# penincillin/IHMR

Hardware: AMD Instinct MI355X
Metric: images/sec, IHMR-OPT 200-iter refinement batch=64 (ms/refine-iter: latency.ms_per_refine_iter; amortised: ms_per_refine_iter_amortised) (higher is better)
Workload: dtype f32

## Files before the change

ihmr_amd/csrc/ihmr_hip.hip:

```cpp
#include <math.h>
#include <stdio.h>
#include <stdlib.h>
#include <string.h>

#include <algorithm>
#include <atomic>
#include <mutex>
#include <vector>

#include "ihmr_common.h"
#include "mano_lbs.h"
#include "sdf_collision.h"
#include "preprocess.h"
#include "augment.h"
#include "render.h"
#include "mlp_infer.h"
#include "refine.h"
#include "encoder.h"
#include "encoder_bf16.h"
#include "evaluate.h"
#include "train.h"
#include "train_conv.h"
#include "copy_pack.h"
#include "launch_plan.h"
// ... 105 lines not shown
        jseg[j] = (int32_t)seg_q.size();
        for (int q = start[j]; q < start[j + 1]; q += LBS_SEG) seg_q.push_back(q);
    }
    jseg[NJ] = (int32_t)seg_q.size();
    seg_q.push_back((int32_t)wv.size());
    std::vector<int32_t> fsoa((size_t)3 * NFP, 0);
    for (int f = 0; f < NFP; ++f)
        for (int k = 0; k < 3; ++k) {
            const int32_t id = h->faces[(f < NF ? f : 0) * 3 + k];
            if (id < 0 || id >= NV) { delete m; return -1; }
            fsoa[(size_t)k * NFP + f] = id;
        }
    std::vector<uint32_t> fpk(NFP, 0u);
    for (int f = 0; f < NFP; ++f)
        fpk[f] = (uint32_t)fsoa[f] | ((uint32_t)fsoa[(size_t)NFP + f] << 10) | ((uint32_t)fsoa[(size_t)2 * NFP + f] << 20);
    std::vector<float> pd4, sd4, vt4;
    pack4(pd.data(), NPF, pd4);
    pack4(sd_t.data(), 10, sd4);
    pack4(vt.data(), 1, vt4);
    int rc = 0;
    rc |= upload_as(&m->pd4, pd4); rc |= upload_as(&m->sd4, sd4); rc |= upload_as(&m->vt4, vt4);
    rc |= upload(&m->v_template, vt); rc |= upload(&m->shapedirs_t, sd_t); rc |= upload(&m->posedirs, pd);
    rc |= upload(&m->J_template, J_t); rc |= upload(&m->J_shapedirs, J_sd); rc |= upload(&m->weights, wts);
    rc |= upload_as(&m->w4_w, w4w); rc |= upload(&m->w4_j, w4j);
    m->sparse4 = sparse4;
    rc |= upload(&m->pose_mean, pm); rc |= upload(&m->parents, par); rc |= upload(&m->depth, depth);
    rc |= upload(&m->tip_ids, tips); rc |= upload(&m->wj_start, start); rc |= upload(&m->wj_vert, wv);
    rc |= upload(&m->wj_w, ww); rc |= upload(&m->seg_q, seg_q); rc |= upload(&m->jseg_start, jseg); rc |= upload(&m->faces, fsoa); rc |= upload(&m->faces_pk, fpk); rc |= upload(&m->J_regressor, jr);
    m->max_depth = maxd;
    m->nnz = (int)wv.size();
    m->nseg = (int)seg_q.size() - 1;
    if (m->nseg > LBS_SEG_CAP) { ihmr_mano_destroy(m); return -1; }
    {
        const int dyn = m->nseg * 12 * (int)sizeof(float);
        hipError_t e1 = hipFuncSetAttribute((const void*)lbs_bwd1_kernel<true>, hipFuncAttributeMaxDynamicSharedMemorySize, dyn);
        hipError_t e2 = hipFuncSetAttribute((const void*)lbs_bwd1_kernel<false>, hipFuncAttributeMaxDynamicSharedMemorySize, dyn);
        if (e1 != hipSuccess || e2 != hipSuccess) { ihmr_mano_destroy(m); return (int)(e1 != hipSuccess ? e1 : e2); }
        int dev = 0, lds_max = 0;
        (void)hipGetDevice(&dev);
        (void)hipDeviceGetAttribute(&lds_max, hipDeviceAttributeMaxSharedMemoryPerBlock, dev);
        const void* tails[4] = {(const void*)opt_tail_kernel<true, true>, (const void*)opt_tail_kernel<true>, (const void*)opt_tail_kernel<false>,
                                (const void*)opt_tail_kernel_trans};
        m->tail_fits = 1;
        const int tail_dyn = opt_tail_dynamic_lds(m->nseg);
        for (const void* k : tails) {
            hipFuncAttributes fa;
            const int dyn_k = k == (const void*)opt_tail_kernel_trans ? 0 : tail_dyn;
            if (hipFuncGetAttributes(&fa, k) != hipSuccess || (long)fa.sharedSizeBytes + dyn_k > (long)lds_max ||
                (dyn_k && hipFuncSetAttribute(k, hipFuncAttributeMaxDynamicSharedMemorySize, dyn_k) != hipSuccess))
                m->tail_fits = 0;
        }
        (void)hipGetLastError();
    }
    if (rc) return rc;
    *out = m;
    return 0;
}

extern "C" int ihmr_mano_destroy(ihmr_mano* m) {
    if (!m) return 0;
    void* ptrs[] = {m->v_template, m->shapedirs_t, m->posedirs, m->J_template, m->J_shapedirs, m->weights, m->pose_mean,
                    m->parents, m->depth, m->tip_ids, m->wj_start, m->wj_vert, m->wj_w, m->faces, m->J_regressor, m->pd4, m->sd4, m->vt4, m->seg_q, m->jseg_start,
                    m->w4_w, m->w4_j, m->faces_pk};
    for (void* p : ptrs)
        if (p) (void)hipFree(p);
    delete m;
    return 0;
}

extern "C" int ihmr_mano_update_shapedirs(ihmr_mano* m, const float* shapedirs_host) {
    if (!m || !shapedirs_host) return -1;
    std::vector<float> jr((size_t)NJ * NV), vt(NV3), sd_t, J_t, J_sd;
    HIP_TRY(hipMemcpy(jr.data(), m->J_regressor, jr.size() * 4, hipMemcpyDeviceToHost));
    HIP_TRY(hipMemcpy(vt.data(), m->v_template, vt.size() * 4, hipMemcpyDeviceToHost));
    derive_shape_constants(jr.data(), vt.data(), shapedirs_host, sd_t, J_t, J_sd);
    HIP_TRY(hipMemcpy(m->shapedirs_t, sd_t.data(), sd_t.size() * 4, hipMemcpyHostToDevice));
    HIP_TRY(hipMemcpy(m->J_shapedirs, J_sd.data(), J_sd.size() * 4, hipMemcpyHostToDevice));
    std::vector<float> sd4;
    pack4(sd_t.data(), 10, sd4);
    HIP_TRY(hipMemcpy(m->sd4, sd4.data(), sd4.size() * 4, hipMemcpyHostToDevice));
    return 0;
}

extern "C" size_t ihmr_mano_workspace_bytes(int N) { return lbs_ws_bytes(N); }

static_assert(plan::SKIN_SMALL_MAX_HANDS == LBS_SMALL_MAX_HANDS && plan::BWD2_LDS_MIN_HANDS == LBS_B2_MIN_HANDS &&
              plan::PREP_SMALL_MAX_HANDS == SDF_PREP_SMALL_MAX_HANDS, "stage_plan.h restates the launch-form thresholds of the kernel headers");
template <bool TWO_HAND, int MODE>
static void lbs_skin_launch_mode(const ihmr_mano* m, int N, int B, float* verts, float* joints, const LbsWork& wk, float* pose_off, hipStream_t st) {
    const bool small = plan::skin_small(N);
    const int hg8 = 8 * (small ? LBS_HG_SMALL : LBS_HG);
    const dim3 skin_grid(8, 4 * ((N + hg8 - 1) / hg8));
    if (small) hipLaunchKernelGGL((lbs_skin_kernel<TWO_HAND, MODE, LBS_HG_SMALL>), skin_grid, dim3(LBS_THREADS), 0, st, *m, (const float*)wk.skel, N, B,
                                  verts, joints, wk.v_posed, pose_off);
    else hipLaunchKernelGGL((lbs_skin_kernel<TWO_HAND, MODE, LBS_HG>), skin_grid, dim3(LBS_THREADS), 0, st, *m, (const float*)wk.skel, N, B, verts,
                            joints, wk.v_posed, pose_off);
}
#define LBS_SKIN_FULL 0
#define LBS_SKIN_REUSE 1
#define LBS_SKIN_KEEP_P 2
#define LBS_SKIN_FULL_STORE_P 3
static_assert(plan::SKIN_FULL == LBS_SKIN_FULL && plan::SKIN_REUSE == LBS_SKIN_REUSE && plan::SKIN_KEEP_P == LBS_SKIN_KEEP_P &&
              plan::SKIN_FULL_STORE_P == LBS_SKIN_FULL_STORE_P, "stage_plan.h restates the skin modes");
static int g_force_full_skin = 0;
template <bool TWO_HAND>
static void lbs_skin_launch(const ihmr_mano* m, int mode, int N, int B, float* verts, float* joints, const LbsWork& wk, hipStream_t st) {
    if (g_force_full_skin && (mode == LBS_SKIN_KEEP_P || mode == LBS_SKIN_FULL_STORE_P)) mode = LBS_SKIN_FULL;
    if (mode == LBS_SKIN_REUSE) lbs_skin_launch_mode<TWO_HAND, LBS_MODE_REUSE>(m, N, B, verts, joints, wk, nullptr, st);
    else if (mode == LBS_SKIN_KEEP_P) lbs_skin_launch_mode<TWO_HAND, LBS_MODE_KEEP_P>(m, N, B, verts, joints, wk, wk.pose_off, st);
    else lbs_skin_launch_mode<TWO_HAND, LBS_MODE_FULL>(m, N, B, verts, joints, wk, mode == LBS_SKIN_FULL_STORE_P ? wk.pose_off : nullptr, st);
}
extern "C" int ihmr_debug_force_full_skin(int force) {
    const int prev = g_force_full_skin;
    g_force_full_skin = force ? 1 : 0;
    return prev;
}
static int g_force_generic_tail = 0;
extern "C" int ihmr_debug_force_generic_tail(int force) {
    const int prev = g_force_generic_tail;
    g_force_generic_tail = force ? 1 : 0;
    return prev;
}

static void lbs_forward_launch(const ihmr_mano* m, bool two_hand, const float* orient, const float* pose, const float* betas,
                               const float* trans, int N, int B, float* verts, float* joints, const LbsWork& wk, hipStream_t st) {
    if (two_hand) {
        hipLaunchKernelGGL(lbs_skel_kernel<true>, dim3(N), dim3(192), 0, st, *m, orient, pose, betas, trans, B, wk.skel, joints);
        lbs_skin_launch<true>(m, LBS_SKIN_FULL, N, B, verts, joints, wk, st);
    } else {
        hipLaunchKernelGGL(lbs_skel_kernel<false>, dim3(N), dim3(192), 0, st, *m, orient, pose, betas, trans, B, wk.skel, joints);
        lbs_skin_launch<false>(m, LBS_SKIN_FULL, N, B, verts, joints, wk, st);
    }
}

static int g_bwd2_streaming = 0;
extern "C" int ihmr_debug_force_lbs_bwd2_streaming(int force) {
    const int prev = g_bwd2_streaming;
    g_bwd2_streaming = force ? 1 : 0;
    return prev;
}

static void lbs_backward_launch(const ihmr_mano* m, bool two_hand, int N, int B, const float* d_verts, const float* d_joints,
                                float* d_orient, float* d_pose, float* d_betas, float* d_trans, int need_mask, const LbsWork& wk,
                                hipStream_t st, bool bwd1_done = false) {
    const size_t part_lds = (size_t)m->nseg * 12 * sizeof(float);
    if (bwd1_done) {}
    else if (two_hand)
        hipLaunchKernelGGL(lbs_bwd1_kernel<true>, dim3(N), dim3(LBS_THREADS), part_lds, st, *m, wk, B, d_verts, d_joints, d_orient,
                           d_betas, d_trans, need_mask);
    else
        hipLaunchKernelGGL(lbs_bwd1_kernel<false>, dim3(N), dim3(LBS_THREADS), part_lds, st, *m, wk, B, d_verts, d_joints, d_orient,
                           d_betas, d_trans, need_mask);
    if (need_mask & 2) {
        if (plan::bwd2_lds(N, g_bwd2_streaming)) hipLaunchKernelGGL(lbs_bwd2_lds_kernel, dim3((N + 63) / 64, LBS_KG), dim3(320), 0, st, *m, wk, N);
        else hipLaunchKernelGGL(lbs_bwd2_kernel, dim3(5, (N + 31) / 32, LBS_KG), dim3(64), 0, st, *m, wk, N);
        if (two_hand) hipLaunchKernelGGL(lbs_bwd3_kernel<true>, dim3(N), dim3(64), 0, st, wk, N, B, d_pose);
        else hipLaunchKernelGGL(lbs_bwd3_kernel<false>, dim3(N), dim3(64), 0, st, wk, N, B, d_pose);
    }
}

extern "C" int ihmr_mano_lbs_fwd(const ihmr_mano* m, const float* orient, const float* pose, const float* betas, int N,
                                 float* verts, float* joints, void* workspace, void* stream) {
    if (!m || N <= 0 || !workspace) return -1;
    lbs_forward_launch(m, false, orient, pose, betas, nullptr, N, 0, verts, joints, lbs_carve(workspace, N), (hipStream_t)stream);
    return (int)hipGetLastError();
}

extern "C" int ihmr_mano_lbs_bwd(const ihmr_mano* m, int N, const void* workspace, const float* d_verts, const float* d_joints,
                                 float* d_orient, float* d_pose, float* d_betas, int need_mask, void* stream) {
    if (!m || N <= 0 || !workspace) return -1;
    lbs_backward_launch(m, false, N, 0, d_verts, d_joints, d_orient, d_pose, d_betas, nullptr, need_mask,
                        lbs_carve(const_cast<void*>(workspace), N), (hipStream_t)stream);
    return (int)hipGetLastError();
}

static int device_cu_count(int* cus_out) {
    static std::atomic<int> cache[64];
    int dev = 0;
    HIP_TRY(hipGetDevice(&dev));
    int cus = cache[dev & 63].load(std::memory_order_relaxed);
    if (cus == 0) {
        HIP_TRY(hipDeviceGetAttribute(&cus, hipDeviceAttributeMultiprocessorCount, dev));
        if (cus <= 0) cus = 256;
        cache[dev & 63].store(cus, std::memory_order_relaxed);
    }
    *cus_out = cus;
    return 0;
}

extern "C" size_t ihmr_sdf_workspace_bytes(int B) { return sdf_ws_bytes(2 * B) + (size_t)2 * NFP * 4 * 4 + 256; }

static int g_collect_stats = 0;

static int sdf_launch(const VertLayout& vl, const int32_t* faces_r_soa, const int32_t* faces_l_soa, const uint32_t* fpk_r,
                      const uint32_t* fpk_l, int B, SdfWorkspace ws, float robustifier, float* loss, float* per_vert, float* origin, float* dval, bool dense, hipStream_t st) {
    if (B <= 0 || 2 * B > SDF_MAX_HANDS) return -1;
    const int prep = plan::prep_form(2 * B, dense);
    ws.fpk[0] = fpk_r; ws.fpk[1] = fpk_l; ws.B = B;
    const bool timed = g_timer != nullptr;
    hipEvent_t tcur;
    if (timed) { if (int rc = timed_begin(&tcur, st)) return rc; }
    if (prep == plan::PREP_DENSE)
        hipLaunchKernelGGL((sdf_prep_kernel<true, SDF_PREP_THREADS_LARGE>), dim3(2 * B), dim3(SDF_PREP_THREADS_LARGE), 0, st, vl, B, faces_r_soa,
                           faces_l_soa, ws, g_collect_stats);
    else if (prep == plan::PREP_SMALL)
        hipLaunchKernelGGL((sdf_prep_kernel<false, SDF_PREP_THREADS_SMALL>), dim3(2 * B), dim3(SDF_PREP_THREADS_SMALL), 0, st, vl, B, faces_r_soa,
                           faces_l_soa, ws, g_collect_stats);
    else
        hipLaunchKernelGGL((sdf_prep_kernel<false, SDF_PREP_THREADS_LARGE>), dim3(2 * B), dim3(SDF_PREP_THREADS_LARGE), 0, st, vl, B, faces_r_soa,
                           faces_l_soa, ws, g_collect_stats);
    int cus = 0;
    if (int rc = device_cu_count(&cus)) return rc;
    const int dist_blocks = SDF_DIST_WG_PER_CU * cus;
    if (timed) { if (int rc = timed_next(&tcur, IHMR_TIMED_SDF_PREP, st)) return rc; }
    int nblk = dist_blocks;
#ifdef IHMR_TUNING_BUILD
    if (const char* e = getenv("IHMR_DIST_BLOCKS_PER_SAMPLE")) nblk = std::max(64, std::min(dist_blocks, atoi(e) * B));
#endif
    if (g_collect_stats) hipLaunchKernelGGL(sdf_dist_kernel<true>, dim3(nblk), dim3(SDF_THREADS), 0, st, ws);
    else hipLaunchKernelGGL(sdf_dist_kernel<false>, dim3(nblk), dim3(SDF_THREADS), 0, st, ws);
    if (timed) { if (int rc = timed_next(&tcur, IHMR_TIMED_SDF_DIST, st)) return rc; (void)hipEventDestroy(tcur); }
    if (loss)
        hipLaunchKernelGGL(sdf_sample_kernel, dim3(B), dim3(SDF_SAMPLE_THREADS), 0, st, vl, ws, robustifier, loss, per_vert, origin,
                           dval, B);
    return (int)hipGetLastError();
}

__global__ void faces_to_soa_kernel(const int32_t* __restrict__ aos, int32_t* __restrict__ soa, uint32_t* __restrict__ packed, int* zero8) {
    if (zero8 && blockIdx.x == 0 && threadIdx.x < SDF_NZERO) sdf_zero_counter(zero8, (int)threadIdx.x);
    const int f = blockIdx.x * blockDim.x + threadIdx.x;
    if (f >= NFP) return;
    const int s = f < NF ? f : 0;
    uint32_t pk = 0;
    for (int k = 0; k < 3; ++k) {
        const int32_t id = min(max(aos[s * 3 + k], 0), NV - 1);
        soa[k * NFP + f] = id;
        pk |= (uint32_t)id << (10 * k);
    }
    packed[f] = pk;
}
struct FaceCopies { const int32_t *soa_r, *soa_l; const uint32_t *pk_r, *pk_l; };
static FaceCopies faces_to_workspace(const int32_t* faces_right, const int32_t* faces_left, void* workspace, int B, const SdfWorkspace& ws, hipStream_t st) {
    int32_t* soa = (int32_t*)((char*)workspace + sdf_ws_bytes(2 * B));
    uint32_t* pk = (uint32_t*)(soa + 6 * NFP);
    hipLaunchKernelGGL(faces_to_soa_kernel, dim3((NFP + 255) / 256), dim3(256), 0, st, faces_right, soa, pk, ws.inside_count);
    hipLaunchKernelGGL(faces_to_soa_kernel, dim3((NFP + 255) / 256), dim3(256), 0, st, faces_left, soa + 3 * NFP, pk + NFP, (int*)nullptr);
    return FaceCopies{soa, soa + 3 * NFP, pk, pk + NFP};
}

extern "C" int ihmr_sdf_collision_ex(const int32_t* faces_right, const int32_t* faces_left, const float* hand_verts, int B,
                                     float robustifier, const ihmr_sdf_options* options, float* loss, float* per_vert,
                                     float* origin_scale, float* dval, void* workspace, void* stream) {
    if (!workspace || B <= 0 || 2 * B > SDF_MAX_HANDS) return -1;
    hipStream_t st = (hipStream_t)stream;
    SdfWorkspace ws = sdf_carve(workspace, 2 * B);
    if (options) {
        ws.align_corners = options->align_corners ? 1 : 0;
        if (options->loss_divisor > 0.f) ws.loss_div = options->loss_divisor;
        ws.swap_xz = options->swap_xz ? 1 : 0;
    }
    const FaceCopies f = faces_to_workspace(faces_right, faces_left, workspace, B, ws, st);
    VertLayout vl{hand_verts, (long)2 * NV3, (long)NV3};
    return sdf_launch(vl, f.soa_r, f.soa_l, f.pk_r, f.pk_l, B, ws, robustifier, loss, per_vert, origin_scale, dval, false, st);
}

extern "C" int ihmr_sdf_collision(const int32_t* faces_right, const int32_t* faces_left, const float* hand_verts, int B,
                                  float robustifier, float* loss, float* per_vert, float* origin_scale, float* dval,
                                  void* workspace, void* stream) {
    return ihmr_sdf_collision_ex(faces_right, faces_left, hand_verts, B, robustifier, nullptr, loss, per_vert, origin_scale, dval,
                                 workspace, stream);
}

extern "C" int ihmr_sdf_dense_grid(const int32_t* faces_right, const int32_t* faces_left, const float* hand_verts, int B,
                                   float* phi, void* workspace, void* stream) {
    if (!workspace || B <= 0 || 2 * B > SDF_MAX_HANDS) return -1;
    hipStream_t st = (hipStream_t)stream;
    SdfWorkspace ws = sdf_carve(workspace, 2 * B);
    const FaceCopies f = faces_to_workspace(faces_right, faces_left, workspace, B, ws, st);
    VertLayout vl{hand_verts, (long)2 * NV3, (long)NV3};
    int rc = sdf_launch(vl, f.soa_r, f.soa_l, f.pk_r, f.pk_l, B, ws, 0.f, nullptr, nullptr, nullptr, nullptr, true, st);
    if (rc) return rc;
    for (int b = 0; b < B; ++b)
        for (int hnd = 0; hnd < 2; ++hnd)
            HIP_TRY(hipMemcpyAsync(phi + ((size_t)b * 2 + hnd) * SDF_NVOX, ws.phi + ((size_t)hnd * B + b) * SDF_NVOX,
                                   (size_t)SDF_NVOX * 4, hipMemcpyDeviceToDevice, st));
    return (int)hipGetLastError();
}

extern "C" size_t ihmr_opt_workspace_bytes(int B) { return opt_ws_bytes(B); }

static const ParamStep kNoStep{0, 0.f, 0.f, 1.f, -1, 0, 0};
static SdfWorkspace opt_sdf_ws(const ihmr_opt_io* io, const OptWork& wk, int B, int lists, int static_mask) {
    SdfWorkspace ws = sdf_carve(wk.sdf_ws, 2 * B, true);
    const plan::SdfFlags f = plan::plan_sdf_flags(lists, static_mask, io->sdf_no_candidate_lists, io->sdf_no_static_reuse);
    ws.list_mode = f.list_mode;
    ws.force_rebuild = f.force_rebuild;
    ws.static_stage = f.static_stage;
    ws.static_mask = f.static_mask;
    ws.moving_box = f.moving_box;
    ws.align_corners = io->sdf_align_corners ? 1 : 0;
    if (io->sdf_loss_divisor > 0.f) ws.loss_div = io->sdf_loss_divisor;
    ws.swap_xz = io->sdf_swap_xz ? 1 : 0;
    return ws;
}

struct OptCtx {
    const ihmr_mano *m, *m_left;
// ... 656 lines not shown
}

extern "C" int ihmr_render_meshes(const float* verts, const int32_t* faces, const int32_t* csr_offsets, const int32_t* csr_ids, int n_verts,
                                  int n_faces, int face_split, const uint8_t* present, const float* albedo, const float* cam,
                                  const ihmr_render_lights* lights, const uint8_t* background, int S, uint8_t* out_img,
                                  int32_t* out_face_ids, void* workspace, int B, void* stream) {
    if (!verts || !faces || !csr_offsets || !csr_ids || !albedo || !cam || !lights || !out_img || !workspace) return -1;
    if (B <= 0 || B > 65535 || n_verts <= 0 || n_faces <= 0 || n_faces > (1 << 24) || n_verts > (1 << 24) || face_split < 0 ||
        face_split > n_faces || S < 16 || S > 2048)
        return -1;
    if ((uintptr_t)workspace & 3u) return -1;
    const hipStream_t st = (hipStream_t)stream;
    rnd_vertex* ws = static_cast<rnd_vertex*>(workspace);
    hipLaunchKernelGGL(render_vertex_kernel, dim3((n_verts + RND_THREADS - 1) / RND_THREADS, B), dim3(RND_THREADS), 0, st, verts, faces,
                       csr_offsets, csr_ids, n_verts, n_faces, face_split, albedo, cam, *lights, S, ws);
    const int tiles = (S + RND_TILE - 1) / RND_TILE;
    const int vec = S % RND_PPT == 0 && !((uintptr_t)out_img & 3u) && !((uintptr_t)background & 3u);
    hipLaunchKernelGGL(render_raster_kernel, dim3(tiles * tiles, B), dim3(RND_THREADS), 0, st, ws, faces, n_verts, n_faces, face_split,
                       present, background, S, vec, out_img, out_face_ids);
    return (int)hipGetLastError();
}

extern "C" int ihmr_draw_keypoints(uint8_t* img, const float* kps, const float* weight, const uint8_t* colour, int B, int S, int K,
                                   void* stream) {
    if (!img || !kps || !weight || !colour || B <= 0 || S <= 0 || S > 4096 || K <= 0) return -1;
    hipLaunchKernelGGL(draw_keypoints_kernel, dim3(B), dim3(RND_KP_THREADS), 0, (hipStream_t)stream, img, kps, weight, (int)colour[0],
                       (int)colour[1], (int)colour[2], S, K);
    return (int)hipGetLastError();
}

extern "C" int ihmr_copy_segments(const ihmr_copy_seg* segs, int n, void* stream) {
    if (!segs || n <= 0 || n > IHMR_COPY_MAX_SEGS) return -1;
    CopySegTable t;
    memset(&t, 0, sizeof(t));
    long biggest = 0;
    for (int i = 0; i < n; ++i) {
        const ihmr_copy_seg& g = segs[i];
        if (!g.src || !g.dst || g.rows <= 0 || g.width <= 0 || g.src_ld < g.width || g.dst_ld < g.width) return -1;
        if (((uintptr_t)g.src | (uintptr_t)g.dst) & 3u) return -1;
        t.s[i] = g;
        biggest = std::max(biggest, (long)g.rows * g.width);
    }
    const unsigned bx = (unsigned)std::max<long>(1, std::min<long>(64, (biggest + 1023) / 1024));
    hipLaunchKernelGGL(copy_segments_kernel, dim3(bx, (unsigned)n), dim3(256), 0, (hipStream_t)stream, t);
    return (int)hipGetLastError();
}

extern "C" int ihmr_root_align_joints(const float* joints4, float* out4, int B, void* stream) {
    if (!joints4 || !out4 || B <= 0) return -1;
    hipLaunchKernelGGL(root_align_joints_kernel, dim3(B), dim3(64), 0, (hipStream_t)stream, joints4, out4, B);
    return (int)hipGetLastError();
}

extern "C" int ihmr_set_kernel_timer(ihmr_kernel_timer* t) {
    std::lock_guard<std::mutex> lk(g_timer_mutex);
    g_timer = t;
    return 0;
}

extern "C" int ihmr_flush_kernel_timer(void) {
    std::lock_guard<std::mutex> lk(g_timer_mutex);
    for (auto& p : g_pending) {
        float ms = 0.f;
        HIP_TRY(hipEventSynchronize(p.b));
        HIP_TRY(hipEventElapsedTime(&ms, p.a, p.b));
        if (g_timer) {
            if (p.k < 0) { g_timer->ms_event_pair += ms; g_timer->n_event_pair += 1; }
            else if (p.k < IHMR_TIMED_KERNELS) { g_timer->ms[p.k] += ms; g_timer->n[p.k] += 1; }
        }
        (void)hipEventDestroy(p.a);
        (void)hipEventDestroy(p.b);
    }
    g_pending.clear();
    return 0;
}


#ifdef SDF_STAMPS
extern "C" int ihmr_debug_stamps(long long* host, int zero) {
    HIP_TRY(hipDeviceSynchronize());
    if (zero) {
        void* p; HIP_TRY(hipGetSymbolAddress(&p, HIP_SYMBOL(g_sdf_stamps))); HIP_TRY(hipMemset(p, 0, sizeof(long long) * 4096 * 4 * 8));
        HIP_TRY(hipGetSymbolAddress(&p, HIP_SYMBOL(g_sdf_prep))); HIP_TRY(hipMemset(p, 0, sizeof(long long) * 4096 * 8));
        return 0;
    }
    HIP_TRY(hipMemcpyFromSymbol(host, HIP_SYMBOL(g_sdf_stamps), sizeof(long long) * 4096 * 4 * 8));
    HIP_TRY(hipMemcpyFromSymbol(host + 4096 * 4 * 8, HIP_SYMBOL(g_sdf_span), sizeof(long long) * 4096 * 4 * 4));
    HIP_TRY(hipMemcpyFromSymbol(host + 4096 * 4 * 12, HIP_SYMBOL(g_sdf_prep), sizeof(long long) * 4096 * 8));
    return 0;
}
#endif

#ifdef SDF_QMASK_CHECK
extern "C" int ihmr_debug_sdf_ptrs(const ihmr_opt_io* io, int B, void** out4) {
    SdfWorkspace ws = sdf_carve(opt_carve(io->workspace, B).sdf_ws, 2 * B, true);
    out4[0] = ws.qcell; out4[1] = ws.inside_bits; out4[2] = ws.box; out4[3] = ws.phi;
    return 0;
}
extern "C" int ihmr_debug_qmask(unsigned* host8) {
    if (hipDeviceSynchronize() != hipSuccess) return -1;
    return (int)hipMemcpyFromSymbol(host8, HIP_SYMBOL(g_qmask_bad), 32);
}
#endif

#ifdef SDF_HANDLOG
extern "C" long ihmr_debug_handlog(unsigned* host, long cap) {
    static uint4* buf = nullptr;
    static unsigned cap_now = 0;
    if (hipDeviceSynchronize() != hipSuccess) return -1;
    if (cap > 0) {
        if (buf) (void)hipFree(buf);
        if (hipMalloc(&buf, (size_t)cap * 16) != hipSuccess) return -1;
        cap_now = (unsigned)cap;
        const unsigned zero = 0;
        if (hipMemcpyToSymbol(HIP_SYMBOL(g_handlog_n), &zero, 4) != hipSuccess) return -1;
        if (hipMemcpyToSymbol(HIP_SYMBOL(g_handlog_cap), &cap_now, 4) != hipSuccess) return -1;
        if (hipMemcpyToSymbol(HIP_SYMBOL(g_handlog), &buf, 8) != hipSuccess) return -1;
        return 0;
    }
    unsigned n = 0;
    if (hipMemcpyFromSymbol(&n, HIP_SYMBOL(g_handlog_n), 4) != hipSuccess) return -1;
    if (n > cap_now) n = cap_now;
    if (n && hipMemcpy(host, buf, (size_t)n * 16, hipMemcpyDeviceToHost) != hipSuccess) return -1;
    uint4* null = nullptr;
    (void)hipMemcpyToSymbol(HIP_SYMBOL(g_handlog), &null, 8);
    return (long)n;
}
#endif

#ifdef CONV_STAMPS
extern "C" int ihmr_debug_conv_stamps(long long* host, int zero) {
    HIP_TRY(hipDeviceSynchronize());
    void* p;
    HIP_TRY(hipGetSymbolAddress(&p, HIP_SYMBOL(g_conv_stamps)));
    if (zero) { HIP_TRY(hipMemset(p, 0, sizeof(long long) * 1024 * 10)); return 0; }
    HIP_TRY(hipMemcpy(host, p, sizeof(long long) * 1024 * 10, hipMemcpyDeviceToHost));
    return 0;
}
#endif

#ifdef TAIL_STAMPS
extern "C" int ihmr_debug_tail_stamps(long long* host, int zero) {
    HIP_TRY(hipDeviceSynchronize());
    void *p, *q;
    HIP_TRY(hipGetSymbolAddress(&p, HIP_SYMBOL(g_tail_stamps)));
    HIP_TRY(hipGetSymbolAddress(&q, HIP_SYMBOL(g_samp_stamps)));
    if (zero) { HIP_TRY(hipMemset(p, 0, sizeof(long long) * 3 * 4096 * 8)); HIP_TRY(hipMemset(q, 0, sizeof(long long) * 4096 * 8)); return 0; }
    HIP_TRY(hipMemcpy(host, p, sizeof(long long) * 3 * 4096 * 8, hipMemcpyDeviceToHost));
    HIP_TRY(hipMemcpy(host + 3 * 4096 * 8, q, sizeof(long long) * 4096 * 8, hipMemcpyDeviceToHost));
    return 0;
}
#endif

#ifdef IHMR_TIMELINE
extern "C" long ihmr_debug_timeline(unsigned long long* host, long cap) {
    static unsigned long long* ring = nullptr;
    static unsigned seg_cap = 0;
    if (hipDeviceSynchronize() != hipSuccess) return -1;
    void* cur = nullptr;
    if (hipGetSymbolAddress(&cur, HIP_SYMBOL(g_tl_cursor)) != hipSuccess) return -1;
    if (cap > 0) {
        if (ring) (void)hipFree(ring);
        seg_cap = (unsigned)(cap / 256);
        if (hipMalloc(&ring, (size_t)seg_cap * 256 * 24) != hipSuccess) return -1;
        if (hipMemset(cur, 0, 256 * 32 * 4) != hipSuccess) return -1;
        if (hipMemcpyToSymbol(HIP_SYMBOL(g_tl_cap), &seg_cap, 4) != hipSuccess) return -1;
        if (hipMemcpyToSymbol(HIP_SYMBOL(g_tl_ring), &ring, 8) != hipSuccess) return -1;
        return 0;
    }
    static unsigned counts[256 * 32];
    if (hipMemcpy(counts, cur, sizeof(counts), hipMemcpyDeviceToHost) != hipSuccess) return -1;
    long n = 0;
    for (int s = 0; s < 256; ++s) {
        const unsigned c = counts[s * 32] < seg_cap ? counts[s * 32] : seg_cap;
        if (c && hipMemcpy(host + 3 * n, ring + 3 * (size_t)s * seg_cap, (size_t)c * 24, hipMemcpyDeviceToHost) != hipSuccess) return -1;
        n += c;
    }
    unsigned long long* null = nullptr;
    (void)hipMemcpyToSymbol(HIP_SYMBOL(g_tl_ring), &null, 8);
    return n;
}
#endif

extern "C" const char* ihmr_version(void) { return "ihmr_hip 0.2 (gfx950)"; }
```

ihmr_amd/csrc/mano_lbs.h:

```cpp
#pragma once
#include "ihmr_common.h"

#define LBS_THREADS 256
#define LBS_HG 8
#define LBS_HG_SMALL 4
#define LBS_SMALL_MAX_HANDS 256
#define LBS_TILE_V 195
#define LBS_KG 25
#define LBS_KC 3
#define LBS_SEG 13
#define LBS_SEG_CAP 1024
#define LBS_CSR_CAP 4096

#define SK_R 0
#define SK_J 144
#define SK_G 192
#define SK_A 384
#define SK_PF 576
#define SK_POSE 712
#define SK_BETA 760
#define SK_SHIFT 770
#define SK_STRIDE 784

struct LbsWork {
// ... 724 lines not shown
            }
            if (nc > 0) {
                bw.dG[p][e] += acc;
                if (c == 3) bw.dJ[p][r] -= accJ;
            }
        }
        if (tid >= 192 && tid < 192 + NJ * 3) {
            const int j = (tid - 192) / 3, c = (tid - 192) % 3;
            if (bw.dep[j] == d) bw.dJ[j][c] += bw.drel[j][c];
        }
        __syncthreads();
    }
    if (tid < 9) bw.dR[0][tid] = bw.dG[0][4 * (tid / 3) + (tid % 3)];
    if (tid >= 64 && tid < 67) bw.dJ[0][tid - 64] += bw.dG[0][4 * (tid - 64) + 3];
    __syncthreads();

    if (need_orient && tid == 0) {
        float dr[3];
        rodrigues_bwd(bw.sk + SK_POSE, bw.dR[0], dr);
        if (left) { dr[1] = -dr[1]; dr[2] = -dr[2]; }
        d_orient[h * 3 + 0] = dr[0]; d_orient[h * 3 + 1] = dr[1]; d_orient[h * 3 + 2] = dr[2];
    }
    if (need_pose && tid < NJ * 9) wk.chain[(size_t)h * 192 + tid] = bw.dR[tid / 9][tid % 9];

    if (need_betas) {
        if (TWO_HAND) {
            __syncthreads();
            if (tid < 3) {
                if (!left) bw.dJ[0][tid] += bw.gsum[tid];
                else bw.dJ[0][tid] += tid == 0 ? bw.gsum[0] : -bw.gsum[tid];
            }
            __syncthreads();
        }
        const int wave = tid / WAVE, lane = tid % WAVE;
        if (IN_LDS) {
            for (int l = wave; l < 10; l += LBS_THREADS / WAVE) {
                float4 srow[NVP / WAVE];
#pragma unroll
                for (int t = 0; t < NVP / WAVE; ++t) srow[t] = m.sd4[l * NVP + lane + WAVE * t];
                __builtin_amdgcn_sched_barrier(0);
                float acc = 0.f;
#pragma unroll
                for (int t = 0; t < NVP / WAVE; ++t) {
                    const int v = lane + WAVE * t;
                    if (v < NV) {
                        acc = __builtin_fmaf(srow[t].x, bw.vp[3 * v], acc);
                        acc = __builtin_fmaf(srow[t].y, bw.vp[3 * v + 1], acc);
                        acc = __builtin_fmaf(srow[t].z, bw.vp[3 * v + 2], acc);
                    }
                }
                if (lane < 48) acc = __builtin_fmaf(m.J_shapedirs[lane * 10 + l], bw.dJ[lane / 3][lane % 3], acc);
                acc = wave_reduce_sum(acc);
                if (lane == 0) d_betas[h * 10 + l] = acc;
            }
            return;
        }
        const float* dvp_h = wk.dvp + (size_t)h * NV3;
        for (int l = wave; l < 10; l += LBS_THREADS / WAVE) {
            float acc = 0.f;
#pragma unroll
            for (int half = 0; half < 2; ++half) {
                constexpr int T0[2] = {0, 7}, T1[2] = {7, NVP / WAVE};
                float4 srow[7];
                float dv[7][3];
#pragma unroll
                for (int t = T0[half]; t < T1[half]; ++t) {
                    const int v = min(lane + WAVE * t, NV - 1);
                    srow[t - T0[half]] = m.sd4[l * NVP + lane + WAVE * t];
                    dv[t - T0[half]][0] = dvp_h[3 * v]; dv[t - T0[half]][1] = dvp_h[3 * v + 1]; dv[t - T0[half]][2] = dvp_h[3 * v + 2];
                }
                __builtin_amdgcn_sched_barrier(0);
#pragma unroll
                for (int t = T0[half]; t < T1[half]; ++t) {
                    if (lane + WAVE * t < NV) {
                        acc = __builtin_fmaf(srow[t - T0[half]].x, dv[t - T0[half]][0], acc);
                        acc = __builtin_fmaf(srow[t - T0[half]].y, dv[t - T0[half]][1], acc);
                        acc = __builtin_fmaf(srow[t - T0[half]].z, dv[t - T0[half]][2], acc);
                    }
                }
            }
            if (lane < 48) acc = __builtin_fmaf(m.J_shapedirs[lane * 10 + l], bw.dJ[lane / 3][lane % 3], acc);
            acc = wave_reduce_sum(acc);
            if (lane == 0) d_betas[h * 10 + l] = acc;
        }
    }
}

template <bool TWO_HAND>
__global__ __launch_bounds__(LBS_THREADS, 4) void lbs_bwd1_kernel(ihmr_mano m, LbsWork wk, int B,
                                                               const float* __restrict__ d_verts,
                                                               const float* __restrict__ d_joints,
                                                               float* __restrict__ d_orient, float* __restrict__ d_betas,
                                                               float* __restrict__ d_trans, int need_mask) {
    __shared__ LbsBwdShared bw;
    extern __shared__ __attribute__((aligned(16))) float bwd1_part[];
    lbs_bwd1_hand<TWO_HAND>(m, wk, B, (int)blockIdx.x, (int)threadIdx.x, bw, bwd1_part, d_verts, d_joints, d_orient, d_betas, d_trans, need_mask);
}

typedef float lbs_f32x16 __attribute__((ext_vector_type(16)));
__global__ __launch_bounds__(64) void lbs_bwd2_kernel(ihmr_mano m, LbsWork wk, int N) {
    TL_SCOPE(8);
    const int lane = threadIdx.x, l31 = lane & 31, kp = lane >> 5;
    const int e = blockIdx.x * 32 + l31, hand = blockIdx.y * 32 + l31, kg = blockIdx.z;
    const float* arow = m.posedirs + (size_t)min(e, NPF - 1) * NV3;
    const float* brow = wk.dvp + (size_t)min(hand, N - 1) * NV3;
    const bool a_ok = e < NPF, b_ok = hand < N;
    typedef float lbs_f4u __attribute__((ext_vector_type(4), aligned(8)));
    lbs_f4u av[LBS_KC][4], bv[LBS_KC][4];
#pragma unroll
    for (int c = 0; c < LBS_KC; ++c) {
        const int k0 = (kg * LBS_KC + c) * 32 + 16 * kp;
#pragma unroll
        for (int q = 0; q < 4; ++q) {
            const int k = min(k0 + 4 * q, NV3 - 4);
            av[c][q] = *reinterpret_cast<const lbs_f4u*>(arow + k);
            bv[c][q] = *reinterpret_cast<const lbs_f4u*>(brow + k);
        }
    }
    __builtin_amdgcn_sched_barrier(0);
    lbs_f32x16 acc;
#pragma unroll
    for (int r = 0; r < 16; ++r) acc[r] = 0.f;
#pragma unroll
    for (int c = 0; c < LBS_KC; ++c) {
        const int k0 = (kg * LBS_KC + c) * 32 + 16 * kp;
#pragma unroll
        for (int q = 0; q < 4; ++q) {
            const int kq = k0 + 4 * q;
            const bool sh = kq + 4 > NV3 && kq < NV3;
            const float ax[4] = {sh ? av[c][q].z : av[c][q].x, sh ? av[c][q].w : av[c][q].y, av[c][q].z, av[c][q].w};
            const float bx[4] = {sh ? bv[c][q].z : bv[c][q].x, sh ? bv[c][q].w : bv[c][q].y, bv[c][q].z, bv[c][q].w};
#pragma unroll
            for (int t = 0; t < 4; ++t) {
                const bool k_ok = kq + t < NV3;
                const float a0 = (a_ok && k_ok) ? ax[t] : 0.f, b0 = (b_ok && k_ok) ? bx[t] : 0.f;
                acc = __builtin_amdgcn_mfma_f32_32x32x2f32(a0, b0, acc, 0, 0, 0);
            }
        }
    }
    if (b_ok) {
        float* dst = wk.dpf_part + ((size_t)kg * N + hand) * 136 + blockIdx.x * 32 + 4 * kp;
#pragma unroll
        for (int r4 = 0; r4 < 4; ++r4) {
            const int e4 = blockIdx.x * 32 + 4 * kp + 8 * r4;
            if (e4 + 3 < 136) *reinterpret_cast<float4*>(dst + 8 * r4) = make_float4(acc[4 * r4], acc[4 * r4 + 1], acc[4 * r4 + 2], acc[4 * r4 + 3]);
        }
    }
}

#ifndef LBS_B2_MIN_HANDS
#define LBS_B2_MIN_HANDS 256
#endif
#define LBS_B2_LDK 33
#define LBS_B2_ROWS (160 + 64)
__global__ __launch_bounds__(320) void lbs_bwd2_lds_kernel(ihmr_mano m, LbsWork wk, int N) {
    TL_SCOPE(8);
    __shared__ float tile[2][LBS_B2_ROWS][LBS_B2_LDK];
    const int tid = threadIdx.x, lane = tid % WAVE, wave = tid / WAVE, l31 = lane & 31, kp = lane >> 5;
    const int h0 = blockIdx.x * 64, kg = blockIdx.y;
    float v4[6][4];
    auto load_chunk = [&](int c) {
        const int k0 = (kg * LBS_KC + c) * 32;
#pragma unroll
        for (int i = 0; i < 6; ++i) {
            const int u = tid + 320 * i, row = u >> 3, k = k0 + 4 * (u & 7);
            v4[i][0] = v4[i][1] = v4[i][2] = v4[i][3] = 0.f;
            if (row >= LBS_B2_ROWS) continue;
            const bool is_a = row < 160;
            const int r = is_a ? row : h0 + (row - 160);
            if (is_a ? r >= NPF : r >= N) continue;
            const float* src = (is_a ? m.posedirs + (size_t)r * NV3 : wk.dvp + (size_t)r * NV3) + k;
            if (k + 3 < NV3) {
                typedef float lbs_f4u __attribute__((ext_vector_type(4), aligned(4)));
                const lbs_f4u x = *reinterpret_cast<const lbs_f4u*>(src);
                v4[i][0] = x.x; v4[i][1] = x.y; v4[i][2] = x.z; v4[i][3] = x.w;
            } else {
#pragma unroll
                for (int t = 0; t < 4; ++t) v4[i][t] = k + t < NV3 ? src[t] : 0.f;
            }
        }
    };
    auto store_chunk = [&](int buf) {
#pragma unroll
        for (int i = 0; i < 6; ++i) {
            const int u = tid + 320 * i, row = u >> 3, kq = 4 * (u & 7);
            if (row >= LBS_B2_ROWS) continue;
#pragma unroll
            for (int t = 0; t < 4; ++t) tile[buf][row][kq + t] = v4[i][t];
        }
    };
    lbs_f32x16 acc0, acc1;
#pragma unroll
    for (int r = 0; r < 16; ++r) { acc0[r] = 0.f; acc1[r] = 0.f; }
    load_chunk(0);
    store_chunk(0);
    __syncthreads();
#pragma unroll 1
    for (int c = 0; c < LBS_KC; ++c) {
        const int cur = c & 1;
        if (c + 1 < LBS_KC) load_chunk(c + 1);
        const float* arow = &tile[cur][wave * 32 + l31][16 * kp];
        const float* b0row = &tile[cur][160 + l31][16 * kp];
        const float* b1row = &tile[cur][160 + 32 + l31][16 * kp];
#pragma unroll
        for (int st = 0; st < 16; ++st) {
            const float a = arow[st], b0 = b0row[st], b1 = b1row[st];
            acc0 = __builtin_amdgcn_mfma_f32_32x32x2f32(a, b0, acc0, 0, 0, 0);
            acc1 = __builtin_amdgcn_mfma_f32_32x32x2f32(a, b1, acc1, 0, 0, 0);
        }
        if (c + 1 < LBS_KC) store_chunk(cur ^ 1);
        __syncthreads();
    }
#pragma unroll
    for (int half = 0; half < 2; ++half) {
        const int hand = h0 + 32 * half + l31;
        if (hand >= N) continue;
        const lbs_f32x16& acc = half ? acc1 : acc0;
        float* dst = wk.dpf_part + ((size_t)kg * N + hand) * 136 + wave * 32 + 4 * kp;
#pragma unroll
        for (int r4 = 0; r4 < 4; ++r4) {
            const int e4 = wave * 32 + 4 * kp + 8 * r4;
            if (e4 + 3 < 136) *reinterpret_cast<float4*>(dst + 8 * r4) = make_float4(acc[4 * r4], acc[4 * r4 + 1], acc[4 * r4 + 2], acc[4 * r4 + 3]);
        }
    }
}

template <bool TWO_HAND>
__device__ __forceinline__ void lbs_bwd3_hand(const LbsWork& wk, int N, int B, float* __restrict__ d_pose, int h, int j, float* dpf, bool active = true) {
    float r[3] = {0.f, 0.f, 0.f}, chain[9];
    const int jj = min(max(j, 1), NJ - 1);
    if (active) {
#pragma unroll
        for (int t = 0; t < 3; ++t) {
            const int e = j + 64 * t;
            if (e >= 136) break;
            float part[LBS_KG];
#pragma unroll
            for (int c = 0; c < LBS_KG; ++c) part[c] = wk.dpf_part[((size_t)c * N + h) * 136 + e];
            __builtin_amdgcn_sched_barrier(0);
            float acc = 0.f;
#pragma unroll
            for (int c = 0; c < LBS_KG; ++c) acc += part[c];
            dpf[e] = acc;
        }
#pragma unroll
        for (int k = 0; k < 3; ++k) r[k] = wk.skel[(size_t)h * SK_STRIDE + SK_POSE + 3 * jj + k];
#pragma unroll
        for (int e = 0; e < 9; ++e) chain[e] = wk.chain[(size_t)h * 192 + 9 * jj + e];
    }
    __syncthreads();
    if (!active || j < 1 || j >= NJ) return;
    const bool left = TWO_HAND && h >= B;
    float dR[9], dr[3];
#pragma unroll
    for (int e = 0; e < 9; ++e) dR[e] = chain[e] + dpf[(j - 1) * 9 + e];
    rodrigues_bwd(r, dR, dr);
    if (left) { dr[1] = -dr[1]; dr[2] = -dr[2]; }
    float* dst = d_pose + (size_t)h * 45 + 3 * (j - 1);
    dst[0] = dr[0]; dst[1] = dr[1]; dst[2] = dr[2];
}
template <bool TWO_HAND>
__global__ __launch_bounds__(64) void lbs_bwd3_kernel(LbsWork wk, int N, int B, float* __restrict__ d_pose) {
    TL_SCOPE(9);
    __shared__ float dpf[192];
    lbs_bwd3_hand<TWO_HAND>(wk, N, B, d_pose, (int)blockIdx.x, (int)threadIdx.x, dpf);
}
```

Baseline: 29810.

## Retile LBS bwd2 LDS GEMM to 32 hands per block with staged output

Reworks the posedirs-by-dvp GEMM kernel to process 32 hands per workgroup with 4 waves instead of 64 hands with 5 waves. The 8 leftover pose-feature rows are computed by a 16x16x4 MFMA on two waves. Row pointers are precomputed and tail loads are clamped, and results are staged through LDS so the global writes are coalesced. This doubles the grid size for better CU occupancy at small batches, at the cost of re-reading posedirs per block and adding divergent work for the remainder rows.

```diff
diff --git a/ihmr_amd/csrc/ihmr_hip.hip b/ihmr_amd/csrc/ihmr_hip.hip
--- a/ihmr_amd/csrc/ihmr_hip.hip
+++ b/ihmr_amd/csrc/ihmr_hip.hip
@@ -281,7 +281,7 @@
         hipLaunchKernelGGL(lbs_bwd1_kernel<false>, dim3(N), dim3(LBS_THREADS), part_lds, st, *m, wk, B, d_verts, d_joints, d_orient,
                            d_betas, d_trans, need_mask);
     if (need_mask & 2) {
-        if (plan::bwd2_lds(N, g_bwd2_streaming)) hipLaunchKernelGGL(lbs_bwd2_lds_kernel, dim3((N + 63) / 64, LBS_KG), dim3(320), 0, st, *m, wk, N);
+        if (plan::bwd2_lds(N, g_bwd2_streaming)) hipLaunchKernelGGL(lbs_bwd2_lds_kernel, dim3((N + LBS_B2_HANDS - 1) / LBS_B2_HANDS, LBS_KG), dim3(256), 0, st, *m, wk, N);
         else hipLaunchKernelGGL(lbs_bwd2_kernel, dim3(5, (N + 31) / 32, LBS_KG), dim3(64), 0, st, *m, wk, N);
         if (two_hand) hipLaunchKernelGGL(lbs_bwd3_kernel<true>, dim3(N), dim3(64), 0, st, wk, N, B, d_pose);
         else hipLaunchKernelGGL(lbs_bwd3_kernel<false>, dim3(N), dim3(64), 0, st, wk, N, B, d_pose);
@@ -1244,6 +1244,17 @@
 }
 #endif
 
+#ifdef BWD2_STAMPS
+extern "C" int ihmr_debug_bwd2_stamps(long long* host, int zero) {
+    HIP_TRY(hipDeviceSynchronize());
+    void* p;
+    HIP_TRY(hipGetSymbolAddress(&p, HIP_SYMBOL(g_bwd2_stamps)));
+    if (zero) { HIP_TRY(hipMemset(p, 0, sizeof(long long) * 1024 * 8)); return 0; }
+    HIP_TRY(hipMemcpy(host, p, sizeof(long long) * 1024 * 8, hipMemcpyDeviceToHost));
+    return 0;
+}
+#endif
+
 #ifdef IHMR_TIMELINE
 extern "C" long ihmr_debug_timeline(unsigned long long* host, long cap) {
     static unsigned long long* ring = nullptr;
diff --git a/ihmr_amd/csrc/mano_lbs.h b/ihmr_amd/csrc/mano_lbs.h
--- a/ihmr_amd/csrc/mano_lbs.h
+++ b/ihmr_amd/csrc/mano_lbs.h
@@ -900,77 +900,111 @@
 #define LBS_B2_MIN_HANDS 256
 #endif
 #define LBS_B2_LDK 33
-#define LBS_B2_ROWS (160 + 64)
-__global__ __launch_bounds__(320) void lbs_bwd2_lds_kernel(ihmr_mano m, LbsWork wk, int N) {
+#define LBS_B2_HANDS 32
+#define LBS_B2_ROWS (128 + LBS_B2_HANDS + 8)
+#define LBS_B2_OLD 140
+typedef float lbs_f32x4 __attribute__((ext_vector_type(4)));
+#ifdef BWD2_STAMPS
+__device__ long long g_bwd2_stamps[1024][8];
+#define BWD2_TK(k) do { const long long now_ = (long long)__builtin_readcyclecounter(); tk_[k] += now_ - tk_prev_; tk_prev_ = now_; } while (0)
+#else
+#define BWD2_TK(k)
+#endif
+__global__ __launch_bounds__(256) void lbs_bwd2_lds_kernel(ihmr_mano m, LbsWork wk, int N) {
     TL_SCOPE(8);
-    __shared__ float tile[2][LBS_B2_ROWS][LBS_B2_LDK];
-    const int tid = threadIdx.x, lane = tid % WAVE, wave = tid / WAVE, l31 = lane & 31, kp = lane >> 5;
-    const int h0 = blockIdx.x * 64, kg = blockIdx.y;
-    float v4[6][4];
+    __shared__ __attribute__((aligned(16))) float tile[2][LBS_B2_ROWS][LBS_B2_LDK];
+    static_assert(LBS_B2_HANDS * LBS_B2_OLD <= 2 * LBS_B2_ROWS * LBS_B2_LDK, "the output tile reuses the chunk buffers");
+    const int tid = threadIdx.x, lane = tid % WAVE, l31 = lane & 31, kp = lane >> 5;
+    const int wave = __builtin_amdgcn_readfirstlane(tid / WAVE);
+    const int h0 = blockIdx.x * LBS_B2_HANDS, kg = blockIdx.y;
+#ifdef BWD2_STAMPS
+    long long tk_[8] = {0, 0, 0, 0, 0, 0, 0, 0}, tk_prev_ = (long long)__builtin_readcyclecounter();
+#endif
+    typedef float lbs_f4u __attribute__((ext_vector_type(4), aligned(4)));
+    const float* srow[6];
+    bool sok[6];
+#pragma unroll
+    for (int i = 0; i < 6; ++i) {
+        const int row = (tid + 256 * i) >> 3;
+        if (row < 128) { srow[i] = m.posedirs + (size_t)row * NV3; sok[i] = true; }
+        else if (row < 128 + LBS_B2_HANDS) { const int h = h0 + row - 128; srow[i] = wk.dvp + (size_t)min(h, N - 1) * NV3; sok[i] = h < N; }
+        else { const int e = row - LBS_B2_HANDS; srow[i] = m.posedirs + (size_t)min(e, NPF - 1) * NV3; sok[i] = e < NPF; }
+    }
+    lbs_f4u v4[6];
     auto load_chunk = [&](int c) {
-        const int k0 = (kg * LBS_KC + c) * 32;
+        const int k = (kg * LBS_KC + c) * 32 + 4 * (tid & 7), kc = min(k, NV3 - 4);
+#pragma unroll
+        for (int i = 0; i < 6; ++i)
+            if (i < 5 || wave == 0) v4[i] = *reinterpret_cast<const lbs_f4u*>(srow[i] + kc);
+    };
+    auto store_chunk = [&](int buf, int c) {
+        const int k = (kg * LBS_KC + c) * 32 + 4 * (tid & 7);
+        const bool sh = k + 4 > NV3 && k < NV3;
 #pragma unroll
         for (int i = 0; i < 6; ++i) {
-            const int u = tid + 320 * i, row = u >> 3, k = k0 + 4 * (u & 7);
-            v4[i][0] = v4[i][1] = v4[i][2] = v4[i][3] = 0.f;
-            if (row >= LBS_B2_ROWS) continue;
-            const bool is_a = row < 160;
-            const int r = is_a ? row : h0 + (row - 160);
-            if (is_a ? r >= NPF : r >= N) continue;
-            const float* src = (is_a ? m.posedirs + (size_t)r * NV3 : wk.dvp + (size_t)r * NV3) + k;
-            if (k + 3 < NV3) {
-                typedef float lbs_f4u __attribute__((ext_vector_type(4), aligned(4)));
-                const lbs_f4u x = *reinterpret_cast<const lbs_f4u*>(src);
-                v4[i][0] = x.x; v4[i][1] = x.y; v4[i][2] = x.z; v4[i][3] = x.w;
-            } else {
-#pragma unroll
-                for (int t = 0; t < 4; ++t) v4[i][t] = k + t < NV3 ? src[t] : 0.f;
-            }
+            if (i == 5 && wave != 0) continue;
+            const float x[4] = {sh ? v4[i].z : v4[i].x, sh ? v4[i].w : v4[i].y, v4[i].z, v4[i].w};
+            float* dst = &tile[buf][(tid + 256 * i) >> 3][4 * (tid & 7)];
+#pragma unroll
+            for (int t = 0; t < 4; ++t) dst[t] = (sok[i] && k + t < NV3) ? x[t] : 0.f;
         }
     };
-    auto store_chunk = [&](int buf) {
-#pragma unroll
-        for (int i = 0; i < 6; ++i) {
-            const int u = tid + 320 * i, row = u >> 3, kq = 4 * (u & 7);
-            if (row >= LBS_B2_ROWS) continue;
-#pragma unroll
-            for (int t = 0; t < 4; ++t) tile[buf][row][kq + t] = v4[i][t];
-        }
-    };
-    lbs_f32x16 acc0, acc1;
-#pragma unroll
-    for (int r = 0; r < 16; ++r) { acc0[r] = 0.f; acc1[r] = 0.f; }
+    lbs_f32x16 acc;
+    lbs_f32x4 acc7 = {0.f, 0.f, 0.f, 0.f};
+#pragma unroll
+    for (int r = 0; r < 16; ++r) acc[r] = 0.f;
+    const int g16 = lane >> 4, l15 = lane & 15;
     load_chunk(0);
-    store_chunk(0);
-    __syncthreads();
+    store_chunk(0, 0);
+    __syncthreads();
+    BWD2_TK(0);
 #pragma unroll 1
     for (int c = 0; c < LBS_KC; ++c) {
         const int cur = c & 1;
         if (c + 1 < LBS_KC) load_chunk(c + 1);
         const float* arow = &tile[cur][wave * 32 + l31][16 * kp];
-        const float* b0row = &tile[cur][160 + l31][16 * kp];
-        const float* b1row = &tile[cur][160 + 32 + l31][16 * kp];
-#pragma unroll
-        for (int st = 0; st < 16; ++st) {
-            const float a = arow[st], b0 = b0row[st], b1 = b1row[st];
-            acc0 = __builtin_amdgcn_mfma_f32_32x32x2f32(a, b0, acc0, 0, 0, 0);
-            acc1 = __builtin_amdgcn_mfma_f32_32x32x2f32(a, b1, acc1, 0, 0, 0);
-        }
-        if (c + 1 < LBS_KC) store_chunk(cur ^ 1);
+        const float* brow = &tile[cur][128 + l31][16 * kp];
+        if (wave >= 2) {
+            const float* a7row = &tile[cur][128 + LBS_B2_HANDS + (l15 & 7)][16 * (g16 & 1) + (g16 >> 1)];
+            const float* b7row = &tile[cur][128 + 16 * (wave - 2) + l15][16 * (g16 & 1) + (g16 >> 1)];
+#pragma unroll
+            for (int t = 0; t < 8; ++t) {
+                acc = __builtin_amdgcn_mfma_f32_32x32x2f32(arow[2 * t], brow[2 * t], acc, 0, 0, 0);
+                const float a7 = l15 < 8 ? a7row[2 * t] : 0.f;
+                acc7 = __builtin_amdgcn_mfma_f32_16x16x4f32(a7, b7row[2 * t], acc7, 0, 0, 0);
+                acc = __builtin_amdgcn_mfma_f32_32x32x2f32(arow[2 * t + 1], brow[2 * t + 1], acc, 0, 0, 0);
+            }
+        } else {
+#pragma unroll
+            for (int st = 0; st < 16; ++st) acc = __builtin_amdgcn_mfma_f32_32x32x2f32(arow[st], brow[st], acc, 0, 0, 0);
+        }
+        BWD2_TK(1);
+        if (c + 1 < LBS_KC) store_chunk(cur ^ 1, c + 1);
+        BWD2_TK(2);
         __syncthreads();
-    }
-#pragma unroll
-    for (int half = 0; half < 2; ++half) {
-        const int hand = h0 + 32 * half + l31;
-        if (hand >= N) continue;
-        const lbs_f32x16& acc = half ? acc1 : acc0;
-        float* dst = wk.dpf_part + ((size_t)kg * N + hand) * 136 + wave * 32 + 4 * kp;
-#pragma unroll
-        for (int r4 = 0; r4 < 4; ++r4) {
-            const int e4 = wave * 32 + 4 * kp + 8 * r4;
-            if (e4 + 3 < 136) *reinterpret_cast<float4*>(dst + 8 * r4) = make_float4(acc[4 * r4], acc[4 * r4 + 1], acc[4 * r4 + 2], acc[4 * r4 + 3]);
-        }
-    }
+        BWD2_TK(3);
+    }
+    float* out = &tile[0][0][0];
+#pragma unroll
+    for (int r4 = 0; r4 < 4; ++r4)
+        *reinterpret_cast<float4*>(out + l31 * LBS_B2_OLD + wave * 32 + 4 * kp + 8 * r4) = make_float4(acc[4 * r4], acc[4 * r4 + 1], acc[4 * r4 + 2], acc[4 * r4 + 3]);
+    if (wave >= 2 && g16 < 2)
+        *reinterpret_cast<float4*>(out + (16 * (wave - 2) + l15) * LBS_B2_OLD + 128 + 4 * g16) = make_float4(acc7[0], acc7[1], acc7[2], acc7[3]);
+    __syncthreads();
+    BWD2_TK(4);
+    const int n4 = min(LBS_B2_HANDS, N - h0) * 34;
+    float4* dst = reinterpret_cast<float4*>(wk.dpf_part + ((size_t)kg * N + h0) * 136);
+    for (int i = tid; i < n4; i += 256) dst[i] = *reinterpret_cast<const float4*>(out + (i / 34) * LBS_B2_OLD + 4 * (i % 34));
+#ifdef BWD2_STAMPS
+    BWD2_TK(5);
+    if (tid == 0) {
+        const int wg = blockIdx.y * gridDim.x + blockIdx.x;
+        if (wg < 1024) {
+            for (int k = 0; k < 6; ++k) g_bwd2_stamps[wg][k] += tk_[k];
+            g_bwd2_stamps[wg][7] += 1;
+        }
+    }
+#endif
 }
 
 template <bool TWO_HAND>
```

Result: faster. 30210 (median of 6 runs) (+1.3%).
